# yifanlu0227/CoAlign

Hardware: AMD Instinct MI355X
Metric: frames_per_s_5agent_opv2v_synthetic (higher is better)
Workload: dtype f32 (3x3 convolutions: every operand rounded to 22 significant bits and split into two fp16 terms, the low term scaled by 2^10 and the weights by a per-output-channel power of two so that both terms are normal fp16 numbers at any scale; three fp16 matrix products per fp32 product, f32 accumulation

## Files before the change

coalign_amd/backbone.py:

```python
from __future__ import annotations

import os
from collections import namedtuple
from typing import List, Optional, Sequence

import torch
import torch.nn as nn
import torch.nn.functional as F

from . import ops

FAST_INFERENCE = True


def _bn(ch: int, eps: float) -> nn.BatchNorm2d:
    return nn.BatchNorm2d(ch, eps=eps, momentum=0.01)


def _fast_ok(module: nn.Module, x: torch.Tensor) -> bool:
    return FAST_INFERENCE and (not module.training) and x.is_cuda and x.dtype == torch.float32


HIP_CONV_POLICY = os.environ.get("COALIGN_HIP_CONV", "stage1")

# ... 7 lines not shown


def _terms(terms: Optional[int]) -> int:
    return CONV_EMU_TERMS if terms is None else terms


def emu_active(terms: Optional[int] = None) -> bool:
    return _terms(terms) in EMU_MODES

NHWC_STAGE_OUTPUTS = os.environ.get("COALIGN_NHWC_STAGES", "1") != "0"
CONV_EMU_TAP_MAJOR = os.environ.get("COALIGN_EMU_TAPK", "1") != "0"
CONV_WINOGRAD = os.environ.get("COALIGN_WINOGRAD", "0") != "0"


SPLIT_MAPS = os.environ.get("COALIGN_SPLIT_MAPS", "1") != "0"
HEAD_SPLIT_MAPS = os.environ.get("COALIGN_HEAD_SPLIT_MAPS", "1") != "0"


S2_SPLIT = os.environ.get("COALIGN_S2_SP", "all")
S2_SKIP = os.environ.get("COALIGN_S2_SKIP", "1") != "0"


HEADS_ONE_LAUNCH = os.environ.get("COALIGN_HEADS_ONE_LAUNCH", "1") != "0"
HEADS_SPLIT_IN = os.environ.get("COALIGN_HEADS_SP", "1") != "0"
COMPRESS_SPARSE = os.environ.get("COALIGN_COMPRESS_SPARSE", "1") != "0"


def split_maps_active(terms: Optional[int] = None) -> bool:
    return SPLIT_MAPS and _terms(terms) == 16 and NHWC_STAGE_OUTPUTS and CONV_EMU_TAP_MAJOR and POINTWISE_EMU


SP_MAX_COUT, SP_MAX_COUT_SKIP = 1024, 512


def sp_channels_ok(cin: Optional[int], cout: int, skip: bool = False) -> bool:
    return cout % 64 == 0 and 0 < cout <= (SP_MAX_COUT_SKIP if skip else SP_MAX_COUT) and (cin is None or (cin > 0 and cin % 16 == 0))


def narrow_channels_ok(cin: int, cout: int) -> bool:
    return cout in ops.NARROW_COUTS and cin > 0 and cin % 16 == 0


def winograd_active(terms: Optional[int] = None) -> bool:
    return CONV_WINOGRAD and _terms(terms) == 3 and NHWC_STAGE_OUTPUTS


# ... 368 lines not shown

    def _pointwise_ok(self, feats: Sequence[torch.Tensor]) -> bool:
        if not self.heads_pointwise() or not _fast_ok(self, feats[0]):
            return False
        sizes = {(f.shape[0], f.shape[2] * self.deblocks[i][0].stride[0], f.shape[3] * self.deblocks[i][0].stride[0]) for i, f in enumerate(feats[: self.num_levels])}
        return len(sizes) == 1

    def _upsample_concat(self, feats: Sequence[torch.Tensor], out_split: bool = False):
        if self._pointwise_ok(feats):
            ops_, c_tot = [], 0
            for i, f in enumerate(feats[: self.num_levels]):
                blk = self.deblocks[i]
                op, bn = blk[0], blk[1]
                w, b = _cache_of(blk, "_coalign_pw_cache").get(blk, lambda op=op, bn=bn: (lambda wf, bf: (PointwisePack(wf, True), bf))(*fold_bn(op.weight, None, bn, out_dim=1)))
                ops_.append((f, w, b, op.out_channels, op.stride[0], c_tot))
                c_tot += op.out_channels
            f0, s0 = feats[0], self.deblocks[0][0].stride[0]
            images = [w.get() for _, w, _, _, _, _ in ops_]
            if out_split and self.heads_write_split():
                x = ops.SplitMap.empty(f0.shape[0], c_tot, f0.shape[2] * s0, f0.shape[3] * s0, f0.device)
            else:
                x = torch.empty((f0.shape[0], c_tot, f0.shape[2] * s0, f0.shape[3] * s0), dtype=torch.float32, device=f0.device)
            if isinstance(x, ops.SplitMap) and HEADS_ONE_LAUNCH and 1 < len(ops_) <= 4:
                ops.pointwise_heads_split([(f, im, b, cout, up, off) for (f, w, b, cout, up, off), im in zip(ops_, images)], x)
            else:
                for (f, w, b, cout, up, off), im in zip(ops_, images):
                    ops.pointwise_conv(f, im, b, cout, up=up, relu=True, out=x, c_off=off)
        else:
            ups = [self._deblock(i, f) if len(self.deblocks) > 0 else f for i, f in enumerate(feats[: self.num_levels])]
            x = torch.cat(ups, dim=1) if len(ups) > 1 else ups[0]
        if len(self.deblocks) > self.num_levels:
            x = self._deblock(len(self.deblocks) - 1, x)
        return x

    def decode_multiscale_feature(self, feats: Sequence[torch.Tensor], out_split: bool = False):
        return self._upsample_concat(feats, out_split)

    def forward(self, data_dict: dict) -> dict:
        feats = self.get_multiscale_feature(data_dict["spatial_features"])
        data_dict["spatial_features_2d"] = self._upsample_concat(feats)
        return data_dict


def _backbone_cfg(model_cfg: dict):
    layer_nums, layer_strides, num_filters, ups, upf = (list(model_cfg.get(k, [])) for k in ("layer_nums", "layer_strides", "num_filters", "upsample_strides", "num_upsample_filter"))
    assert len(layer_nums) == len(layer_strides) == len(num_filters) and len(ups) == len(upf)
    return layer_nums, layer_strides, num_filters, ups, upf


class ResNetBEVBackbone(_MultiscaleDecodeMixin, nn.Module):
# ... 192 lines not shown
```

coalign_amd/csrc/pointwise.hip:

```cpp
#include "common.h"
#include <cstdlib>

namespace {

typedef float floatx16 __attribute__((ext_vector_type(16)));

constexpr int kMaxCin = 256;

struct PwArgs {
    const float *__restrict__ x, *__restrict__ w, *__restrict__ bias;
    float *__restrict__ y;
    int N, Cin, Hin, Win, in_stride, Hp, Wp, M, up, Cout, Ctot, c_off, relu;
    int in_nhwc;
    int pb;
    int out_nhwc;
    const unsigned long long *stamps;
    const int *tag_ptr;
    unsigned sparse_rows;
    int out_sp;
    int *range_flag;
};

template <int UP>
__device__ __forceinline__ void pw_store(const PwArgs &a, int n, int m0, bool second, int px, int half, const floatx16 &acc0, const floatx16 &acc1) {
    const int pixels = a.Hp * a.Wp;
    if (px >= pixels) return;
    const int hp = px / a.Wp, wp = px - hp * a.Wp;
    const int Ho = a.Hp * UP, Wo = a.Wp * UP;
    const size_t out_plane = (size_t)Ho * Wo;
    float *yout = a.y + ((size_t)n * a.Ctot + a.c_off) * out_plane;
#pragma unroll
    for (int t = 0; t < 2; ++t) {
        if (t == 1 && !second) break;
#pragma unroll
        for (int r4 = 0; r4 < 4; ++r4) {
            const int m = m0 + t * 32 + 8 * r4 + 4 * half;
            float v[4];
#pragma unroll
            for (int j = 0; j < 4; ++j) v[j] = t == 0 ? acc0[4 * r4 + j] : acc1[4 * r4 + j];
            if (UP == 4) {
                const int co = m >> 4, ky = (m >> 2) & 3;
                const float bb = a.bias[co];
                float4 o;
                o.x = v[0] + bb; o.y = v[1] + bb; o.z = v[2] + bb; o.w = v[3] + bb;
// ... 76 lines not shown
        }
    }
    __syncthreads();
    const int pbk = wave / WPB, rt = wave - pbk * WPB;
    const int m0 = m_base + rt * 64;
    const bool active = m0 < a.M;
    if (!active && !a.out_sp) return;
    const bool second = m0 + 32 < a.M;
    floatx16 acc0 = {0}, acc1 = {0};
    const float *w0 = a.w + m0 + p;
    const float *xb = xt + pbk * 32 + p;
#pragma unroll 8
    for (int k0 = 0; k0 < a.Cin; k0 += 2) {
        const float b = xb[(k0 + half) * TP];
        const float a0 = w0[(size_t)(k0 + half) * a.M];
        const float a1 = second ? w0[(size_t)(k0 + half) * a.M + 32] : 0.f;
        acc0 = __builtin_amdgcn_mfma_f32_32x32x2f32(a0, b, acc0, 0, 0, 0);
        acc1 = __builtin_amdgcn_mfma_f32_32x32x2f32(a1, b, acc1, 0, 0, 0);
    }
    pw_store<UP>(a, n, m0, second, p0 + pbk * 32 + p, half, acc0, acc1);
}

template <int UP>
__device__ __forceinline__ void pw_store_sp(const PwArgs &a, float *stage, int n, int m_base, int p0, int RW, int PB, int tid, int pbk, int rt, int lane, bool active, bool second,
                                            const floatx16 &acc0, const floatx16 &acc1) {
    constexpr int UU = UP * UP;
    const int half = lane >> 5, p = lane & 31;
    __syncthreads();
    if (active) {
#pragma unroll
        for (int t = 0; t < 2; ++t) {
            if (t == 1 && !second) break;
#pragma unroll
            for (int r = 0; r < 16; ++r) {
                const int row = rt * 64 + t * 32 + 8 * (r / 4) + 4 * half + r % 4;
                stage[(pbk * RW + row) * 33 + p] = t == 0 ? acc0[r] : acc1[r];
            }
        }
    }
    __syncthreads();
    const int pixels = a.Hp * a.Wp, Ho = a.Hp * UP, Wo = a.Wp * UP;
    const size_t HWo = (size_t)Ho * Wo;
    const int c8n = RW / (8 * UU);
    const int items = PB * c8n * UU * 32;
    uint4 *ysp = reinterpret_cast<uint4 *>(a.y);
    bool big = false;
    for (int it = tid; it < items; it += 256) {
        const int kx = it % UP, pp = (it / UP) & 31;
        int rest = it / (32 * UP);
        const int ky = rest % UP;
        rest /= UP;
        const int c8 = rest % c8n, pb = rest / c8n;
        const int co0 = m_base / UU + 8 * c8;
        const int px = p0 + pb * 32 + pp;
        if (co0 >= a.Cout || px >= pixels) continue;
        const int hp = px / a.Wp, wp = px - hp * a.Wp;
        const float4 b0 = *reinterpret_cast<const float4 *>(a.bias + co0), b1 = *reinterpret_cast<const float4 *>(a.bias + co0 + 4);
        const float bb[8] = {b0.x, b0.y, b0.z, b0.w, b1.x, b1.y, b1.z, b1.w};
        float v[8];
#pragma unroll
        for (int j = 0; j < 8; ++j) {
            v[j] = stage[(pb * RW + (8 * c8 + j) * UU + ky * UP + kx) * 33 + pp] + bb[j];
            if (a.relu) v[j] = fmaxf(v[j], 0.f);
            big = big || fabsf(v[j]) > 65504.f;
        }
        unsigned h[4], l[4];
#pragma unroll
        for (int k = 0; k < 4; ++k) coalign::sp16_split2(v[2 * k], v[2 * k + 1], h[k], l[k]);
        const int cg = a.c_off + co0;
        const size_t idx = ((size_t)(n * (a.Ctot / 16) + cg / 16) * 4 + ((cg >> 3) & 1) * 2) * HWo + (size_t)(hp * UP + ky) * Wo + wp * UP + kx;
        ysp[idx] = uint4{h[0], h[1], h[2], h[3]};
        ysp[idx + HWo] = uint4{l[0], l[1], l[2], l[3]};
    }
    if (a.range_flag && big) atomicOr(a.range_flag, 1);
}

typedef __bf16 bf16x8 __attribute__((ext_vector_type(8)));

__device__ __forceinline__ void split8(const float (&v)[8], bf16x8 (&out)[3]) {
#pragma unroll
    for (int i = 0; i < 8; ++i) {
        const __bf16 h = (__bf16)v[i];
        const float r = v[i] - (float)h;
        const __bf16 m = (__bf16)r;
        out[0][i] = h; out[1][i] = m; out[2][i] = (__bf16)(r - (float)m);
    }
}

template <int UP>
__device__ __forceinline__ void pointwise_emu_body(const PwArgs &a, uint4 *xs, int bx, int by, int bz) {
    const int tid = threadIdx.x, wave = tid >> 6, lane = tid & 63, half = lane >> 5, p = lane & 31;
    const int pixels = a.Hp * a.Wp;
    const int PB = a.pb, WPB = 4 / PB, TP = 32 * PB;
    const int p0 = bx * TP, n = bz;
    const int m_base = by * (64 * WPB);
    const size_t in_plane = (size_t)a.Hin * a.Win;
    const float *xin = a.stamps ? a.x : a.x + (size_t)n * a.Cin * in_plane;
    const int G = a.Cin >> 3;
    {
        const int pl = tid & (TP - 1), g0 = tid / TP, gstep = 256 / TP;
        const int px = p0 + pl;
        const bool ok0 = px < pixels;
        const int hp = ok0 ? px / a.Wp : 0, wp = ok0 ? px - hp * a.Wp : 0;
        size_t off = (size_t)(hp * a.in_stride) * a.Win + (size_t)wp * a.in_stride;
        bool ok = ok0;
        if (a.stamps) {
            const unsigned long long st = a.stamps[(size_t)n * in_plane + off];
            ok = ok0 && (unsigned)(st >> 32) == (unsigned)*a.tag_ptr && (unsigned)st < a.sparse_rows;
            off = ok ? (size_t)(unsigned)st : 0;
        }
        for (int g = g0; g < G; g += gstep) {
            float u[8];
            if (a.in_nhwc) {
                const float4 *xp = reinterpret_cast<const float4 *>(xin + off * a.Cin) + 2 * g;
                const float4 q0 = xp[0], q1 = xp[1];
                u[0] = q0.x; u[1] = q0.y; u[2] = q0.z; u[3] = q0.w; u[4] = q1.x; u[5] = q1.y; u[6] = q1.z; u[7] = q1.w;
            } else {
#pragma unroll
                for (int j = 0; j < 8; ++j) u[j] = xin[(size_t)(8 * g + j) * in_plane + off];
            }
            if (!ok) {
#pragma unroll
                for (int j = 0; j < 8; ++j) u[j] = 0.f;
            }
            bf16x8 o[3];
            split8(u, o);
#pragma unroll
            for (int t = 0; t < 3; ++t) xs[(t * G + g) * TP + pl] = __builtin_bit_cast(uint4, o[t]);
        }
    }
    __syncthreads();
    const int pbk = wave / WPB, rt = wave - pbk * WPB;
    const int m0 = m_base + rt * 64;
    const bool active = m0 < a.M;
    if (!active && !a.out_sp) return;
    const bool second = m0 + 32 < a.M;
    const int S = a.Cin >> 4;
    const uint4 *w0 = reinterpret_cast<const uint4 *>(a.w) + (size_t)((active ? m0 : 0) >> 5) * S * 192 + lane;
    const uint4 *w1 = w0 + (second ? (size_t)S * 192 : 0);
    const uint4 *xb = xs + pbk * 32 + p;
    floatx16 acc0 = {0}, acc1 = {0};
    constexpr int wi[6] = {0, 1, 2, 0, 1, 0};
    constexpr int bi[6] = {2, 1, 0, 1, 0, 0};
    bf16x8 wa[3], wb[3], bc[3];
#pragma unroll
    for (int t = 0; t < 3; ++t) {
        wa[t] = __builtin_bit_cast(bf16x8, w0[t * 64]);
        wb[t] = __builtin_bit_cast(bf16x8, w1[t * 64]);
        bc[t] = __builtin_bit_cast(bf16x8, xb[(t * G + half) * TP]);
    }
    const int steps = active ? S : 0;
#pragma unroll 2
    for (int s = 0; s < steps; ++s) {
        bf16x8 na[3], nb[3], nc[3];
        const int sn = s + 1 < S ? s + 1 : s;
#pragma unroll
        for (int t = 0; t < 3; ++t) {
            na[t] = __builtin_bit_cast(bf16x8, w0[(sn * 3 + t) * 64]);
            nb[t] = __builtin_bit_cast(bf16x8, w1[(sn * 3 + t) * 64]);
            nc[t] = __builtin_bit_cast(bf16x8, xb[(t * G + 2 * sn + half) * TP]);
        }
#pragma unroll
        for (int i = 0; i < 6; ++i) {
            acc0 = __builtin_amdgcn_mfma_f32_32x32x16_bf16(wa[wi[i]], bc[bi[i]], acc0, 0, 0, 0);
            acc1 = __builtin_amdgcn_mfma_f32_32x32x16_bf16(wb[wi[i]], bc[bi[i]], acc1, 0, 0, 0);
        }
#pragma unroll
        for (int t = 0; t < 3; ++t) { wa[t] = na[t]; wb[t] = nb[t]; bc[t] = nc[t]; }
    }
    if (a.out_sp) pw_store_sp<UP>(a, reinterpret_cast<float *>(xs), n, m_base, p0, 64 * WPB, PB, tid, pbk, rt, lane, active, second, acc0, acc1);
    else pw_store<UP>(a, n, m0, second, p0 + pbk * 32 + p, half, acc0, acc1);
}

template <int UP>
__global__ __launch_bounds__(256) void pointwise_emu_kernel(const PwArgs a) {
    extern __shared__ uint4 xs[];
    pointwise_emu_body<UP>(a, xs, blockIdx.x, blockIdx.y, blockIdx.z);
}

constexpr int kMultiMax = 4;
struct PwMulti {
    PwArgs l[kMultiMax];
    int first[kMultiMax + 1], gx[kMultiMax], gy[kMultiMax];
    int n;
};

__global__ __launch_bounds__(256) void pointwise_emu_multi_kernel(const PwMulti m) {
    extern __shared__ uint4 xs[];
    const int bid = blockIdx.x;
#define COALIGN_PW_SLOT(K)                                                                  \
    if (bid >= m.first[K] && bid < m.first[K + 1]) {                                        \
        const PwArgs &a = m.l[K];                                                           \
        const int local = bid - m.first[K], gx = m.gx[K], gy = m.gy[K];                     \
        const int bx = local % gx, by = (local / gx) % gy, bz = local / (gx * gy);          \
        if (a.up == 4) pointwise_emu_body<4>(a, xs, bx, by, bz);                            \
        else if (a.up == 2) pointwise_emu_body<2>(a, xs, bx, by, bz);                       \
        else pointwise_emu_body<1>(a, xs, bx, by, bz);                                      \
        return;                                                                             \
    }
    COALIGN_PW_SLOT(0)
    COALIGN_PW_SLOT(1)
    COALIGN_PW_SLOT(2)
    COALIGN_PW_SLOT(3)
#undef COALIGN_PW_SLOT
}

}

extern "C" int coalign_pointwise_conv(const float *x, const float *w, const float *bias, float *y, int N, int Cin, int Hin, int Win,
                                      int in_stride, int Cout, int up, int M_padded, int Ctot, int c_off, int relu, void *stream) {
    return coalign_pointwise_conv_ex(x, w, bias, y, N, Cin, Hin, Win, in_stride, Cout, up, M_padded, Ctot, c_off, relu, 0, stream);
}

static int pointwise_prepare(const float *x, const float *w, const float *bias, float *y, int N, int Cin, int Hin, int Win,
                             int in_stride, int Cout, int up, int M_padded, int Ctot, int c_off, int relu, int in_nhwc, bool emu,
                             const void *stamps, const int32_t *state, bool out_sp, int32_t *range_flag, int sparse_rows, PwArgs &a, dim3 &grid, size_t &lds) {
    using namespace coalign;
    if (!x || !w || !bias || !y) return COALIGN_ERR_NULL_POINTER;
    if (emu && ((Cin & 15) || (reinterpret_cast<uintptr_t>(w) & 15))) return COALIGN_ERR_UNSUPPORTED;
    if (N < 0 || Cin < 1 || Hin < 1 || Win < 1 || Cout < 1 || Ctot < Cout || c_off < 0 || c_off + Cout > Ctot) return COALIGN_ERR_BAD_SHAPE;
    if ((in_nhwc & 1) && ((Cin & 3) || (reinterpret_cast<uintptr_t>(x) & 15))) return COALIGN_ERR_UNSUPPORTED;
    if (Cin > (emu ? 2 * kMaxCin : kMaxCin) || (Cin & 1) || (up != 1 && up != 2 && up != 4) || (in_stride != 1 && in_stride != 2) || (up != 1 && in_stride != 1))
        return COALIGN_ERR_UNSUPPORTED;
    const int M = Cout * up * up;
    if (M_padded < M || M_padded % 32 || (up != 1 && M_padded != M)) return COALIGN_ERR_BAD_SHAPE;
    const int out_nhwc = (in_nhwc >> 1) & 1;
    in_nhwc &= 1;
    if (out_nhwc && (up != 1 || (Ctot & 3) || (c_off & 3) || ((reinterpret_cast<uintptr_t>(y) | reinterpret_cast<uintptr_t>(bias)) & 15))) return COALIGN_ERR_UNSUPPORTED;
    a = PwArgs{x, w, bias, y, N, Cin, Hin, Win, in_stride, (Hin + in_stride - 1) / in_stride, (Win + in_stride - 1) / in_stride, M_padded, up, Cout, Ctot, c_off, relu, in_nhwc != 0, 1, out_nhwc,
               static_cast<const unsigned long long *>(stamps), state, (unsigned)(sparse_rows < 0 ? 0 : sparse_rows), out_sp ? 1 : 0, range_flag};
    if (out_sp && (!emu || out_nhwc || (Cout & 15) || (Ctot & 15) || (c_off & 15) || (reinterpret_cast<uintptr_t>(y) & 15) || (reinterpret_cast<uintptr_t>(bias) & 15) ||
                   M_padded != Cout * up * up || (size_t)N * Ctot * a.Hp * up * a.Wp * up >= ((size_t)1 << 33)))
        return COALIGN_ERR_UNSUPPORTED;
    if (stamps && (!in_nhwc || !state || (reinterpret_cast<uintptr_t>(stamps) & 7))) return COALIGN_ERR_UNSUPPORTED;
    if (N > 65535) return COALIGN_ERR_UNSUPPORTED;
    const int pixels = a.Hp * a.Wp;
    static const int pb_max = coalign::lab_env("COALIGN_PW_PB", 4);
    a.pb = M_padded <= 64 ? 4 : M_padded <= 128 ? 2 : 1;
    while (a.pb > 1 && (a.pb > pb_max || Cin * 32 * a.pb > kMaxCin * 32)) a.pb >>= 1;
    if (up == 4 && ((a.Wp * 4) % 4 || (reinterpret_cast<uintptr_t>(y) & 15))) return COALIGN_ERR_UNSUPPORTED;
    if (up == 2 && (reinterpret_cast<uintptr_t>(y) & 7)) return COALIGN_ERR_UNSUPPORTED;
    const int rows_per_wg = 64 * (4 / a.pb), px_per_wg = 32 * a.pb;
    grid = dim3((pixels + px_per_wg - 1) / px_per_wg, (M_padded + rows_per_wg - 1) / rows_per_wg, N);
    lds = 0;
    if (emu) {
        lds = (size_t)Cin * px_per_wg * 6;
        if (out_sp && lds < (size_t)256 * 33 * 4) lds = (size_t)256 * 33 * 4;
    }
    return COALIGN_OK;
}

static int pointwise_big_lds(size_t lds) {
    using namespace coalign;
    static bool big_lds_dev[16] = {false};
    int dev = 0;
    if (hipGetDevice(&dev) != hipSuccess || dev < 0 || dev >= 16) dev = 0;
    bool &big_lds = big_lds_dev[dev];
    if (lds > 48 * 1024 && !big_lds) {
        const void *fns[4] = {reinterpret_cast<const void *>(pointwise_emu_kernel<1>), reinterpret_cast<const void *>(pointwise_emu_kernel<2>),
                              reinterpret_cast<const void *>(pointwise_emu_kernel<4>), reinterpret_cast<const void *>(pointwise_emu_multi_kernel)};
        for (const void *fn : fns) {
            const int rc = hip_call(hipFuncSetAttribute(fn, hipFuncAttributeMaxDynamicSharedMemorySize, 96 * 1024));
            if (rc != COALIGN_OK) {
                (void)hipGetLastError();
                return rc;
            }
        }
        big_lds = true;
    }
    return COALIGN_OK;
}

static int pointwise_impl(const float *x, const float *w, const float *bias, float *y, int N, int Cin, int Hin, int Win,
                          int in_stride, int Cout, int up, int M_padded, int Ctot, int c_off, int relu, int in_nhwc, bool emu,
                          void *stream, const void *stamps = nullptr, const int32_t *state = nullptr, bool out_sp = false, int32_t *range_flag = nullptr, int sparse_rows = 0) {
    using namespace coalign;
    PwArgs a;
    dim3 grid;
    size_t lds;
    int rc = pointwise_prepare(x, w, bias, y, N, Cin, Hin, Win, in_stride, Cout, up, M_padded, Ctot, c_off, relu, in_nhwc, emu, stamps, state, out_sp, range_flag, sparse_rows, a, grid, lds);
    if (rc != COALIGN_OK) return rc;
    if (N == 0) return COALIGN_OK;
    hipStream_t s = static_cast<hipStream_t>(stream);
    if (emu) {
        rc = pointwise_big_lds(lds);
        if (rc != COALIGN_OK) return rc;
        if (up == 4) hipLaunchKernelGGL(pointwise_emu_kernel<4>, grid, dim3(256), lds, s, a);
        else if (up == 2) hipLaunchKernelGGL(pointwise_emu_kernel<2>, grid, dim3(256), lds, s, a);
        else hipLaunchKernelGGL(pointwise_emu_kernel<1>, grid, dim3(256), lds, s, a);
        return check_launch();
    }
    if (up == 4) hipLaunchKernelGGL(pointwise_kernel<4>, grid, dim3(256), 0, s, a);
    else if (up == 2) hipLaunchKernelGGL(pointwise_kernel<2>, grid, dim3(256), 0, s, a);
    else hipLaunchKernelGGL(pointwise_kernel<1>, grid, dim3(256), 0, s, a);
    return check_launch();
}

extern "C" int coalign_pointwise_conv_ex(const float *x, const float *w, const float *bias, float *y, int N, int Cin, int Hin, int Win,
                                         int in_stride, int Cout, int up, int M_padded, int Ctot, int c_off, int relu, int in_nhwc,
                                         void *stream) {
    return pointwise_impl(x, w, bias, y, N, Cin, Hin, Win, in_stride, Cout, up, M_padded, Ctot, c_off, relu, in_nhwc, false, stream);
}

extern "C" size_t coalign_pointwise_emu_weight_bytes(int Cin, int M_padded) {
    if (Cin < 16 || (Cin & 15) || Cin > 2 * kMaxCin || M_padded < 32 || (M_padded & 31)) return 0;
    return (size_t)M_padded * Cin * 6;
}

extern "C" int coalign_pointwise_conv_emu(const float *x, const void *w_split, const float *bias, float *y, int N, int Cin, int Hin, int Win,
                                          int in_stride, int Cout, int up, int M_padded, int Ctot, int c_off, int relu, int in_nhwc,
                                          void *stream) {
    return pointwise_impl(x, static_cast<const float *>(w_split), bias, y, N, Cin, Hin, Win, in_stride, Cout, up, M_padded, Ctot, c_off, relu, in_nhwc,
                          true, stream);
}

extern "C" int coalign_pointwise_conv_emu_sparse(const float *feats, int M_rows, const void *stamps, const int32_t *state, const void *w_split, const float *bias, float *y,
                                                 int N, int Cin, int Hin, int Win, int Cout, int M_padded, int relu, int out_nhwc, void *stream) {
    if (!stamps || !state) return COALIGN_ERR_NULL_POINTER;
    if (M_rows < 0) return COALIGN_ERR_BAD_SHAPE;
    return pointwise_impl(feats, static_cast<const float *>(w_split), bias, y, N, Cin, Hin, Win, 2, Cout, 1, M_padded, Cout, 0, relu, 1 | (out_nhwc ? 2 : 0), true, stream,
                          stamps, state, false, nullptr, M_rows);
}

extern "C" int coalign_pointwise_conv_emu_sp(const float *x, const void *w_split, const float *bias, void *y_sp, int N, int Cin, int Hin, int Win, int in_stride,
                                             int Cout, int up, int M_padded, int Ctot, int c_off, int relu, int in_nhwc, int32_t *range_flag, void *stream) {
    if (in_nhwc & ~1) return COALIGN_ERR_UNSUPPORTED;
    return pointwise_impl(x, static_cast<const float *>(w_split), bias, static_cast<float *>(y_sp), N, Cin, Hin, Win, in_stride, Cout, up, M_padded, Ctot, c_off, relu, in_nhwc,
                          true, stream, nullptr, nullptr, true, range_flag);
}

extern "C" int coalign_pointwise_conv_emu_sp_multi(int n_layers, const void *const *x, const void *const *w_split, const void *const *bias, const int32_t *Cin, const int32_t *Hin,
                                                   const int32_t *Win, const int32_t *Cout, const int32_t *up, const int32_t *c_off, const int32_t *in_nhwc, void *y_sp, int N, int Ctot,
                                                   int relu, int32_t *range_flag, void *stream) {
    using namespace coalign;
    if (!x || !w_split || !bias || !Cin || !Hin || !Win || !Cout || !up || !c_off || !in_nhwc || !y_sp) return COALIGN_ERR_NULL_POINTER;
    if (n_layers < 1 || n_layers > kMultiMax) return COALIGN_ERR_UNSUPPORTED;
    PwMulti m{};
    m.n = n_layers;
    size_t lds = 0;
    int order[kMultiMax];
    long long work[kMultiMax];
    for (int i = 0; i < n_layers; ++i) {
        if (in_nhwc[i] & ~1) return COALIGN_ERR_UNSUPPORTED;
        if (Hin[i] * up[i] != Hin[0] * up[0] || Win[i] * up[i] != Win[0] * up[0]) return COALIGN_ERR_BAD_SHAPE;
        order[i] = i;
        work[i] = (long long)Cin[i] * Cout[i] * up[i] * up[i];
    }
    for (int i = 0; i < n_layers; ++i)
        for (int j = i + 1; j < n_layers; ++j)
            if (work[order[j]] > work[order[i]]) { const int t = order[i]; order[i] = order[j]; order[j] = t; }
    for (int k = 0; k < n_layers; ++k) {
        const int i = order[k];
        dim3 grid;
        size_t l;
        const int rc = pointwise_prepare(static_cast<const float *>(x[i]), static_cast<const float *>(w_split[i]), static_cast<const float *>(bias[i]), static_cast<float *>(y_sp), N, Cin[i],
                                         Hin[i], Win[i], 1, Cout[i], up[i], Cout[i] * up[i] * up[i], Ctot, c_off[i], relu, in_nhwc[i], true, nullptr, nullptr, true, range_flag, 0, m.l[k], grid, l);
        if (rc != COALIGN_OK) return rc;
        m.gx[k] = (int)grid.x;
        m.gy[k] = (int)grid.y;
        m.first[k + 1] = m.first[k] + (int)(grid.x * grid.y * grid.z);
        if (l > lds) lds = l;
    }
    for (int k = n_layers; k < kMultiMax; ++k) m.first[k + 1] = m.first[n_layers];
    if (N == 0) return COALIGN_OK;
    const int rc = pointwise_big_lds(lds);
    if (rc != COALIGN_OK) return rc;
    hipLaunchKernelGGL(pointwise_emu_multi_kernel, dim3(m.first[n_layers]), dim3(256), lds, static_cast<hipStream_t>(stream), m);
    return check_launch();
}

namespace {

typedef _Float16 hd_halfx8 __attribute__((ext_vector_type(8)));

struct HeadsArgs {
    const uint4 *__restrict__ x, *__restrict__ w;
    const float *__restrict__ winv, *__restrict__ bias;
    float *__restrict__ y;
    int N, Cin, HW, M;
};

constexpr int kHeadsAhead = 4;

__global__ __launch_bounds__(256) void heads_sp_kernel(const HeadsArgs a) {
    const int tid = threadIdx.x, wave = tid >> 6, lane = tid & 63, half = lane >> 5, p = lane & 31;
    const int n = blockIdx.y, px0 = (blockIdx.x * 4 + wave) * 32;
    if (px0 >= a.HW) return;
    const int px = px0 + p, pix = px < a.HW ? px : a.HW - 1;
    const int CI16 = a.Cin / 16;
    const uint4 *xb = a.x + ((size_t)n * CI16 * 4 + 2 * half) * a.HW + pix;
// ... 50 lines not shown
```

coalign_amd/ops.py:

```python
from __future__ import annotations

import ctypes
import os as _os
from typing import Optional, Sequence, Tuple

import numpy as np
import torch

from . import hip

FUSE_ATT, FUSE_MAX, FUSE_NONE = 0, 1, 2

PROFILE = None


def timed(name: str):
    return _Timed(name)


class _Timed:
    def __init__(self, name: str):
        self.name = name

    def __enter__(self):
# ... 1225 lines not shown
    co, ci = w.shape[0], w.shape[1]
    out = torch.zeros((ci, (co + 31) // 32 * 32), dtype=torch.float32, device=w.device)
    out[:, :co] = w.reshape(co, ci).t()
    return out


def pack_pointwise_emu_weight(w_packed: torch.Tensor) -> torch.Tensor:
    w = w_packed.detach().float()
    Cin, M = w.shape
    if Cin % 16 or M % 32:
        raise ValueError("pointwise emu weights: Cin % 16 == 0 and M % 32 == 0")
    h = w.to(torch.bfloat16)
    r1 = w - h.float()
    m = r1.to(torch.bfloat16)
    lo = (r1 - m.float()).to(torch.bfloat16)
    terms = torch.stack([h, m, lo], 0).view(torch.int16)
    img = terms.view(3, Cin // 16, 2, 8, M // 32, 32)
    img = img.permute(4, 1, 0, 2, 5, 3).contiguous()
    return img.view(M // 32, Cin // 16, 3, 64, 8)


@_device_op
def pointwise_conv(x: torch.Tensor, w_packed: torch.Tensor, bias: torch.Tensor, cout: int, up: int = 1, in_stride: int = 1, relu: bool = True,
                   out: Optional[torch.Tensor] = None, c_off: int = 0, out_channels_last: bool = False) -> torch.Tensor:
    _need_gpu(x, w_packed, bias)
    emu = w_packed.dtype == torch.int16
    L = hip.lib()
    nhwc = x.dtype == torch.float32 and is_channels_last(x) and x.shape[1] % 4 == 0
    xc = x if nhwc else _f32c(x)
    N, Cin, Hin, Win = xc.shape
    Ho, Wo = (Hin + in_stride - 1) // in_stride * up, (Win + in_stride - 1) // in_stride * up
    if isinstance(out, SplitMap):
        if not emu or out_channels_last or tuple(out.shape[2:]) != (Ho, Wo) or out.shape[0] != N or cout % 16 or c_off % 16 or c_off + cout > out.shape[1]:
            raise ValueError("SplitMap output: split-bf16 weight image, [N, Ctot, Ho, Wo] map, Cout and c_off multiples of 16")
        if w_packed.dim() != 5 or w_packed.shape[1] * 16 != Cin or not w_packed.is_contiguous() or w_packed.shape[0] * 32 != cout * up * up:
            raise ValueError("split weight image does not match (Cin, Cout * up * up)")
        with _Timed("pointwise_conv"):
            hip.check(L.coalign_pointwise_conv_emu_sp(_ptr(xc), _ptr(w_packed), _ptr(_f32c(bias)), _ptr(out.data), N, Cin, Hin, Win, in_stride, cout, up, w_packed.shape[0] * 32,
                                                      out.shape[1], c_off, int(relu), int(nhwc), _ptr(sp_range_flag(xc.device)), _stream()), "coalign_pointwise_conv_emu_sp")
        return out
    if out_channels_last:
        if out is not None or up != 1 or cout % 4:
            raise ValueError("channels-last output: up = 1, Cout % 4 == 0, no output slice")
        out = torch.empty((N, cout, Ho, Wo), dtype=torch.float32, device=xc.device, memory_format=torch.channels_last)
    elif out is None:
        out = torch.empty((N, cout, Ho, Wo), dtype=torch.float32, device=xc.device)
    if tuple(out.shape[2:]) != (Ho, Wo) or out.shape[0] != N or not (nhwc_memory(out) if out_channels_last else out.is_contiguous()) or out.dtype != torch.float32:
        raise ValueError("output buffer shape / layout mismatch")
    nhwc_flags = int(nhwc) | (2 if out_channels_last else 0)
    with _Timed("pointwise_conv"):
        if emu:
            if w_packed.dim() != 5 or w_packed.shape[1] * 16 != Cin or not w_packed.is_contiguous():
                raise ValueError("split weight image does not match Cin")
            hip.check(L.coalign_pointwise_conv_emu(_ptr(xc), _ptr(w_packed), _ptr(_f32c(bias)), _ptr(out), N, Cin, Hin, Win, in_stride, cout, up,
                                                   w_packed.shape[0] * 32, out.shape[1], c_off, int(relu), nhwc_flags, _stream()), "coalign_pointwise_conv_emu")
        else:
            hip.check(L.coalign_pointwise_conv_ex(_ptr(xc), _ptr(w_packed), _ptr(_f32c(bias)), _ptr(out), N, Cin, Hin, Win, in_stride, cout, up,
                                                  w_packed.shape[1], out.shape[1], c_off, int(relu), nhwc_flags, _stream()), "coalign_pointwise_conv")
    return out


@_device_op
def pointwise_heads_split(layers, out: "SplitMap", relu: bool = True) -> "SplitMap":
    L = hip.lib()
    n = len(layers)
    N = out.shape[0]
    keep, xs, ws, bs = [], [], [], []
    ci, hi, wi, co, ups, offs, nh = [], [], [], [], [], [], []
    for (x, w_emu, bias, cout, up, c_off) in layers:
        _need_gpu(x, w_emu, bias)
        nhwc = x.dtype == torch.float32 and is_channels_last(x) and x.shape[1] % 4 == 0
        xc = x if nhwc else _f32c(x)
        b = _f32c(bias)
        if w_emu.dtype != torch.int16 or w_emu.dim() != 5 or w_emu.shape[1] * 16 != xc.shape[1] or not w_emu.is_contiguous() or w_emu.shape[0] * 32 != cout * up * up or xc.shape[0] != N:
            raise ValueError("pointwise_heads_split: split weight image of (Cin, Cout * up * up), one batch size")
        keep += [xc, b]
        xs.append(xc.data_ptr()); ws.append(w_emu.data_ptr()); bs.append(b.data_ptr())
        ci.append(xc.shape[1]); hi.append(xc.shape[2]); wi.append(xc.shape[3]); co.append(cout); ups.append(up); offs.append(c_off); nh.append(int(nhwc))
    arr_p = lambda v: (ctypes.c_void_p * n)(*v)
    arr_i = lambda v: (ctypes.c_int32 * n)(*v)
    with _Timed("pointwise_heads_split"):
        hip.check(L.coalign_pointwise_conv_emu_sp_multi(n, arr_p(xs), arr_p(ws), arr_p(bs), arr_i(ci), arr_i(hi), arr_i(wi), arr_i(co), arr_i(ups), arr_i(offs), arr_i(nh), _ptr(out.data),
                                                        N, out.shape[1], int(relu), _ptr(sp_range_flag(out.device)), _stream()), "coalign_pointwise_conv_emu_sp_multi")
    return out


HEADS_SP_MAX_ROWS = 32


def pack_heads_sp_weight(weight: torch.Tensor) -> torch.Tensor:
    w = weight.detach().float().reshape(weight.shape[0], weight.shape[1])
    if w.shape[0] > HEADS_SP_MAX_ROWS:
        raise ValueError("heads_sp serves at most 32 head channels")
    pad = torch.zeros((64, w.shape[1]), dtype=torch.float32, device=w.device)
    pad[: w.shape[0]] = w
    return pack_conv1x1_sp_weight(pad)


@_device_op
def heads_sp(x: "SplitMap", w_sp: torch.Tensor, bias: torch.Tensor, M: int) -> torch.Tensor:
    if not isinstance(x, SplitMap):
# ... 157 lines not shown
```

Before: 691.0.

## Add 2x2 register-tiled pointwise emu kernel with chunked input staging for upsample heads

Adds a new pointwise (1x1/deconv) emulated-fp32 kernel that computes a 2x2 MFMA tile per wave (two row blocks by two pixel blocks), reusing each loaded weight fragment across two pixel groups. It stages input channels into LDS in chunks of KC slices rather than all at once, and is enabled by default for the upsample/concat heads through a flag bit. This raises the arithmetic done per weight load and lowers LDS footprint, at the cost of more accumulator registers and extra barriers between chunks. Optional trace instrumentation macros are also added behind a compile flag.

```diff
diff --git a/coalign_amd/backbone.py b/coalign_amd/backbone.py
--- a/coalign_amd/backbone.py
+++ b/coalign_amd/backbone.py
@@ -53,6 +53,7 @@
 
 
 HEADS_ONE_LAUNCH = os.environ.get("COALIGN_HEADS_ONE_LAUNCH", "1") != "0"
+UPHEADS_TILE = os.environ.get("COALIGN_UPHEADS_TILE", "1") != "0"
 HEADS_SPLIT_IN = os.environ.get("COALIGN_HEADS_SP", "1") != "0"
 COMPRESS_SPARSE = os.environ.get("COALIGN_COMPRESS_SPARSE", "1") != "0"
 
@@ -467,10 +468,10 @@
             else:
                 x = torch.empty((f0.shape[0], c_tot, f0.shape[2] * s0, f0.shape[3] * s0), dtype=torch.float32, device=f0.device)
             if isinstance(x, ops.SplitMap) and HEADS_ONE_LAUNCH and 1 < len(ops_) <= 4:
-                ops.pointwise_heads_split([(f, im, b, cout, up, off) for (f, w, b, cout, up, off), im in zip(ops_, images)], x)
+                ops.pointwise_heads_split([(f, im, b, cout, up, off) for (f, w, b, cout, up, off), im in zip(ops_, images)], x, tile=UPHEADS_TILE)
             else:
                 for (f, w, b, cout, up, off), im in zip(ops_, images):
-                    ops.pointwise_conv(f, im, b, cout, up=up, relu=True, out=x, c_off=off)
+                    ops.pointwise_conv(f, im, b, cout, up=up, relu=True, out=x, c_off=off, tile=UPHEADS_TILE)
         else:
             ups = [self._deblock(i, f) if len(self.deblocks) > 0 else f for i, f in enumerate(feats[: self.num_levels])]
             x = torch.cat(ups, dim=1) if len(ups) > 1 else ups[0]
diff --git a/coalign_amd/csrc/pointwise.hip b/coalign_amd/csrc/pointwise.hip
--- a/coalign_amd/csrc/pointwise.hip
+++ b/coalign_amd/csrc/pointwise.hip
@@ -19,7 +19,48 @@
     unsigned sparse_rows;
     int out_sp;
     int *range_flag;
+    int kc;
+#ifdef PW_TRACE
+    long long *trace;
+    int trace_lds;
+#endif
 };
+
+#ifdef PW_TRACE
+#define PW_TRACE_INIT()                                                                                                          \
+    long long *pw_tr = reinterpret_cast<long long *>(reinterpret_cast<char *>(xs) + a.trace_lds) + wave * 64;                  \
+    const bool pw_on = a.trace && bx == ((pixels + TP - 1) / TP) / 2 && by == 0 && bz == 0;                                      \
+    if (pw_on) pw_tr[lane] = 0
+#define PW_STAMP(k)                                                                                                              \
+    do {                                                                                                                         \
+        unsigned long long pw_t;                                                                                                 \
+        __builtin_amdgcn_sched_barrier(0);                                                                                       \
+        asm volatile("s_memtime %0\n\ts_waitcnt lgkmcnt(0)" : "=s"(pw_t)::"memory");                                            \
+        __builtin_amdgcn_sched_barrier(0);                                                                                       \
+        if (pw_on && lane == 0 && (k) < 64) pw_tr[k] = (long long)pw_t;                                                          \
+    } while (0)
+#define PW_STEP_WAIT(s)                                                                                                          \
+    do {                                                                                                                         \
+        if ((s) < 19) PW_STAMP(2 + 2 * (s));                                                                                     \
+        asm volatile("s_waitcnt vmcnt(6)" ::: "memory");        \
+        if ((s) < 19) PW_STAMP(3 + 2 * (s));                                                                                     \
+    } while (0)
+#define PW_TRACE_FLUSH()                                                                                                         \
+    do {                                                                                                                         \
+        asm volatile("s_waitcnt vmcnt(0)" ::: "memory");                                                                         \
+        PW_STAMP(44);                                                                                                            \
+        if (pw_on) a.trace[((a.up >> 1) * 4 + wave) * 64 + lane] = pw_tr[lane];                                                  \
+    } while (0)
+#define PW_TRACE_PARAMS , bool pw_on, long long *pw_tr
+#define PW_TRACE_ARGS , pw_on, pw_tr
+#else
+#define PW_TRACE_INIT() (void)0
+#define PW_STAMP(k) (void)0
+#define PW_STEP_WAIT(s) (void)0
+#define PW_TRACE_FLUSH() (void)0
+#define PW_TRACE_PARAMS
+#define PW_TRACE_ARGS
+#endif
 
 template <int UP>
 __device__ __forceinline__ void pw_store(const PwArgs &a, int n, int m0, bool second, int px, int half, const floatx16 &acc0, const floatx16 &acc1) {
@@ -142,23 +183,8 @@
 }
 
 template <int UP>
-__device__ __forceinline__ void pw_store_sp(const PwArgs &a, float *stage, int n, int m_base, int p0, int RW, int PB, int tid, int pbk, int rt, int lane, bool active, bool second,
-                                            const floatx16 &acc0, const floatx16 &acc1) {
+__device__ __forceinline__ void pw_sp_groups(const PwArgs &a, const float *stage, int n, int m_base, int p0, int RW, int PB, int tid) {
     constexpr int UU = UP * UP;
-    const int half = lane >> 5, p = lane & 31;
-    __syncthreads();
-    if (active) {
-#pragma unroll
-        for (int t = 0; t < 2; ++t) {
-            if (t == 1 && !second) break;
-#pragma unroll
-            for (int r = 0; r < 16; ++r) {
-                const int row = rt * 64 + t * 32 + 8 * (r / 4) + 4 * half + r % 4;
-                stage[(pbk * RW + row) * 33 + p] = t == 0 ? acc0[r] : acc1[r];
-            }
-        }
-    }
-    __syncthreads();
     const int pixels = a.Hp * a.Wp, Ho = a.Hp * UP, Wo = a.Wp * UP;
     const size_t HWo = (size_t)Ho * Wo;
     const int c8n = RW / (8 * UU);
@@ -195,6 +221,29 @@
     if (a.range_flag && big) atomicOr(a.range_flag, 1);
 }
 
+template <int UP>
+__device__ __forceinline__ void pw_store_sp(const PwArgs &a, float *stage, int n, int m_base, int p0, int RW, int PB, int tid, int pbk, int rt, int lane, bool active, bool second,
+                                            const floatx16 &acc0, const floatx16 &acc1 PW_TRACE_PARAMS) {
+    const int half = lane >> 5, p = lane & 31;
+    __syncthreads();
+    PW_STAMP(41);
+    if (active) {
+#pragma unroll
+        for (int t = 0; t < 2; ++t) {
+            if (t == 1 && !second) break;
+#pragma unroll
+            for (int r = 0; r < 16; ++r) {
+                const int row = rt * 64 + t * 32 + 8 * (r / 4) + 4 * half + r % 4;
+                stage[(pbk * RW + row) * 33 + p] = t == 0 ? acc0[r] : acc1[r];
+            }
+        }
+    }
+    PW_STAMP(42);
+    __syncthreads();
+    PW_STAMP(43);
+    pw_sp_groups<UP>(a, stage, n, m_base, p0, RW, PB, tid);
+}
+
 typedef __bf16 bf16x8 __attribute__((ext_vector_type(8)));
 
 __device__ __forceinline__ void split8(const float (&v)[8], bf16x8 (&out)[3]) {
@@ -217,6 +266,8 @@
     const size_t in_plane = (size_t)a.Hin * a.Win;
     const float *xin = a.stamps ? a.x : a.x + (size_t)n * a.Cin * in_plane;
     const int G = a.Cin >> 3;
+    PW_TRACE_INIT();
+    PW_STAMP(0);
     {
         const int pl = tid & (TP - 1), g0 = tid / TP, gstep = 256 / TP;
         const int px = p0 + pl;
@@ -250,6 +301,7 @@
         }
     }
     __syncthreads();
+    PW_STAMP(1);
     const int pbk = wave / WPB, rt = wave - pbk * WPB;
     const int m0 = m_base + rt * 64;
     const bool active = m0 < a.M;
@@ -278,8 +330,10 @@
         for (int t = 0; t < 3; ++t) {
             na[t] = __builtin_bit_cast(bf16x8, w0[(sn * 3 + t) * 64]);
             nb[t] = __builtin_bit_cast(bf16x8, w1[(sn * 3 + t) * 64]);
-            nc[t] = __builtin_bit_cast(bf16x8, xb[(t * G + 2 * sn + half) * TP]);
-        }
+        }
+        PW_STEP_WAIT(s);
+#pragma unroll
+        for (int t = 0; t < 3; ++t) nc[t] = __builtin_bit_cast(bf16x8, xb[(t * G + 2 * sn + half) * TP]);
 #pragma unroll
         for (int i = 0; i < 6; ++i) {
             acc0 = __builtin_amdgcn_mfma_f32_32x32x16_bf16(wa[wi[i]], bc[bi[i]], acc0, 0, 0, 0);
@@ -288,8 +342,129 @@
 #pragma unroll
         for (int t = 0; t < 3; ++t) { wa[t] = na[t]; wb[t] = nb[t]; bc[t] = nc[t]; }
     }
-    if (a.out_sp) pw_store_sp<UP>(a, reinterpret_cast<float *>(xs), n, m_base, p0, 64 * WPB, PB, tid, pbk, rt, lane, active, second, acc0, acc1);
-    else pw_store<UP>(a, n, m0, second, p0 + pbk * 32 + p, half, acc0, acc1);
+    PW_STAMP(40);
+    if (a.out_sp) {
+        pw_store_sp<UP>(a, reinterpret_cast<float *>(xs), n, m_base, p0, 64 * WPB, PB, tid, pbk, rt, lane, active, second, acc0, acc1 PW_TRACE_ARGS);
+        PW_TRACE_FLUSH();
+    } else {
+        pw_store<UP>(a, n, m0, second, p0 + pbk * 32 + p, half, acc0, acc1);
+    }
+}
+
+template <int UP>
+__device__ __forceinline__ void pointwise_emu_tile_body(const PwArgs &a, uint4 *xs, int bx, int by, int bz) {
+    const int tid = threadIdx.x, wave = tid >> 6, lane = tid & 63, half = lane >> 5, p = lane & 31;
+    const int pixels = a.Hp * a.Wp;
+    const int PP = a.pb, RT = 4 / PP, TP = 64 * PP;
+    const int p0 = bx * TP, n = bz, m_base = by * (64 * RT);
+    const int pq = wave / RT, rt = wave - pq * RT;
+    const int m0 = m_base + rt * 64;
+    const bool active = m0 < a.M, second = m0 + 32 < a.M;
+    const int S = a.Cin >> 4, KC = a.kc, GC = 2 * KC;
+    const size_t in_plane = (size_t)a.Hin * a.Win;
+    const float *xin = a.x + (size_t)n * a.Cin * in_plane;
+    PW_TRACE_INIT();
+    PW_STAMP(0);
+    const int pl = tid & (TP - 1), g0 = tid / TP, gstep = 256 / TP;
+    const bool ok = p0 + pl < pixels;
+    const int hp = ok ? (p0 + pl) / a.Wp : 0, wp = ok ? p0 + pl - hp * a.Wp : 0;
+    const size_t off = (size_t)(hp * a.in_stride) * a.Win + (size_t)wp * a.in_stride;
+    const uint4 *w0 = reinterpret_cast<const uint4 *>(a.w) + (size_t)((active ? m0 : 0) >> 5) * S * 192 + lane;
+    const uint4 *w1 = w0 + (second ? (size_t)S * 192 : 0);
+    const uint4 *xb = xs + pq * 64 + p;
+    floatx16 acc[2][2] = {{{0}, {0}}, {{0}, {0}}};
+    constexpr int wi[6] = {0, 1, 2, 0, 1, 0};
+    constexpr int bi[6] = {2, 1, 0, 1, 0, 0};
+    bf16x8 wa[3], wb[3], bc[2][3];
+#pragma unroll
+    for (int t = 0; t < 3; ++t) {
+        wa[t] = __builtin_bit_cast(bf16x8, w0[t * 64]);
+        wb[t] = __builtin_bit_cast(bf16x8, w1[t * 64]);
+    }
+    for (int s0 = 0; s0 < S; s0 += KC) {
+        const int ns = S - s0 < KC ? S - s0 : KC;
+        if (s0) {
+            if (s0 == KC) PW_STAMP(45);
+            __syncthreads();
+        }
+        for (int g = g0; g < 2 * ns; g += gstep) {
+            float u[8];
+            if (a.in_nhwc) {
+                const float4 *xp = reinterpret_cast<const float4 *>(xin + off * a.Cin) + 2 * (2 * s0 + g);
+                const float4 q0 = xp[0], q1 = xp[1];
+                u[0] = q0.x; u[1] = q0.y; u[2] = q0.z; u[3] = q0.w; u[4] = q1.x; u[5] = q1.y; u[6] = q1.z; u[7] = q1.w;
+            } else {
+#pragma unroll
+                for (int j = 0; j < 8; ++j) u[j] = xin[(size_t)(8 * (2 * s0 + g) + j) * in_plane + off];
+            }
+            if (!ok) {
+#pragma unroll
+                for (int j = 0; j < 8; ++j) u[j] = 0.f;
+            }
+            bf16x8 o[3];
+            split8(u, o);
+#pragma unroll
+            for (int t = 0; t < 3; ++t) xs[(t * GC + g) * TP + pl] = __builtin_bit_cast(uint4, o[t]);
+        }
+        __syncthreads();
+        if (s0 == 0) PW_STAMP(1);
+        if (s0 == KC) PW_STAMP(46);
+        if (!active) continue;
+#pragma unroll
+        for (int t = 0; t < 3; ++t) {
+            bc[0][t] = __builtin_bit_cast(bf16x8, xb[(t * GC + half) * TP]);
+            bc[1][t] = __builtin_bit_cast(bf16x8, xb[(t * GC + half) * TP + 32]);
+        }
+#pragma unroll 2
+        for (int s = 0; s < ns; ++s) {
+            bf16x8 na[3], nb[3], nc[2][3];
+            const int sn = s0 + s + 1 < S ? s0 + s + 1 : s0 + s;
+            const int ln = s + 1 < ns ? s + 1 : s;
+#pragma unroll
+            for (int t = 0; t < 3; ++t) {
+                na[t] = __builtin_bit_cast(bf16x8, w0[(sn * 3 + t) * 64]);
+                nb[t] = __builtin_bit_cast(bf16x8, w1[(sn * 3 + t) * 64]);
+            }
+            PW_STEP_WAIT(s0 + s);
+#pragma unroll
+            for (int t = 0; t < 3; ++t) {
+                nc[0][t] = __builtin_bit_cast(bf16x8, xb[(t * GC + 2 * ln + half) * TP]);
+                nc[1][t] = __builtin_bit_cast(bf16x8, xb[(t * GC + 2 * ln + half) * TP + 32]);
+            }
+#pragma unroll
+            for (int i = 0; i < 6; ++i) {
+                acc[0][0] = __builtin_amdgcn_mfma_f32_32x32x16_bf16(wa[wi[i]], bc[0][bi[i]], acc[0][0], 0, 0, 0);
+                acc[1][0] = __builtin_amdgcn_mfma_f32_32x32x16_bf16(wb[wi[i]], bc[0][bi[i]], acc[1][0], 0, 0, 0);
+                acc[0][1] = __builtin_amdgcn_mfma_f32_32x32x16_bf16(wa[wi[i]], bc[1][bi[i]], acc[0][1], 0, 0, 0);
+                acc[1][1] = __builtin_amdgcn_mfma_f32_32x32x16_bf16(wb[wi[i]], bc[1][bi[i]], acc[1][1], 0, 0, 0);
+            }
+#pragma unroll
+            for (int t = 0; t < 3; ++t) { wa[t] = na[t]; wb[t] = nb[t]; bc[0][t] = nc[0][t]; bc[1][t] = nc[1][t]; }
+        }
+    }
+    PW_STAMP(40);
+    float *stage = reinterpret_cast<float *>(xs);
+    const int RW = 64 * RT;
+    __syncthreads();
+    PW_STAMP(41);
+    if (active) {
+#pragma unroll
+        for (int t = 0; t < 2; ++t) {
+            if (t == 1 && !second) break;
+#pragma unroll
+            for (int q = 0; q < 2; ++q)
+#pragma unroll
+                for (int r = 0; r < 16; ++r) {
+                    const int row = rt * 64 + t * 32 + 8 * (r / 4) + 4 * half + r % 4;
+                    stage[((2 * pq + q) * RW + row) * 33 + p] = acc[t][q][r];
+                }
+        }
+    }
+    PW_STAMP(42);
+    __syncthreads();
+    PW_STAMP(43);
+    pw_sp_groups<UP>(a, stage, n, m_base, p0, RW, 2 * PP, tid);
+    PW_TRACE_FLUSH();
 }
 
 template <int UP>
@@ -308,20 +483,35 @@
 __global__ __launch_bounds__(256) void pointwise_emu_multi_kernel(const PwMulti m) {
     extern __shared__ uint4 xs[];
     const int bid = blockIdx.x;
-#define COALIGN_PW_SLOT(K)                                                                  \
+#define COALIGN_PW_SLOT(K, BODY)                                                            \
     if (bid >= m.first[K] && bid < m.first[K + 1]) {                                        \
         const PwArgs &a = m.l[K];                                                           \
         const int local = bid - m.first[K], gx = m.gx[K], gy = m.gy[K];                     \
         const int bx = local % gx, by = (local / gx) % gy, bz = local / (gx * gy);          \
-        if (a.up == 4) pointwise_emu_body<4>(a, xs, bx, by, bz);                            \
-        else if (a.up == 2) pointwise_emu_body<2>(a, xs, bx, by, bz);                       \
-        else pointwise_emu_body<1>(a, xs, bx, by, bz);                                      \
+        if (a.up == 4) BODY<4>(a, xs, bx, by, bz);                                          \
+        else if (a.up == 2) BODY<2>(a, xs, bx, by, bz);                                     \
+        else BODY<1>(a, xs, bx, by, bz);                                                    \
         return;                                                                             \
     }
-    COALIGN_PW_SLOT(0)
-    COALIGN_PW_SLOT(1)
-    COALIGN_PW_SLOT(2)
-    COALIGN_PW_SLOT(3)
+    COALIGN_PW_SLOT(0, pointwise_emu_body)
+    COALIGN_PW_SLOT(1, pointwise_emu_body)
+    COALIGN_PW_SLOT(2, pointwise_emu_body)
+    COALIGN_PW_SLOT(3, pointwise_emu_body)
+}
+
+template <int UP>
+__global__ __launch_bounds__(256) void pointwise_emu_tile_kernel(const PwArgs a) {
+    extern __shared__ uint4 xs[];
+    pointwise_emu_tile_body<UP>(a, xs, blockIdx.x, blockIdx.y, blockIdx.z);
+}
+
+__global__ __launch_bounds__(256) void pointwise_emu_tile_multi_kernel(const PwMulti m) {
+    extern __shared__ uint4 xs[];
+    const int bid = blockIdx.x;
+    COALIGN_PW_SLOT(0, pointwise_emu_tile_body)
+    COALIGN_PW_SLOT(1, pointwise_emu_tile_body)
+    COALIGN_PW_SLOT(2, pointwise_emu_tile_body)
+    COALIGN_PW_SLOT(3, pointwise_emu_tile_body)
 #undef COALIGN_PW_SLOT
 }
 
@@ -332,9 +522,14 @@
     return coalign_pointwise_conv_ex(x, w, bias, y, N, Cin, Hin, Win, in_stride, Cout, up, M_padded, Ctot, c_off, relu, 0, stream);
 }
 
+#ifdef PW_TRACE
+static long long *g_pw_trace = nullptr;
+extern "C" void coalign_pointwise_set_trace(long long *p) { g_pw_trace = p; }
+#endif
+
 static int pointwise_prepare(const float *x, const float *w, const float *bias, float *y, int N, int Cin, int Hin, int Win,
                              int in_stride, int Cout, int up, int M_padded, int Ctot, int c_off, int relu, int in_nhwc, bool emu,
-                             const void *stamps, const int32_t *state, bool out_sp, int32_t *range_flag, int sparse_rows, PwArgs &a, dim3 &grid, size_t &lds) {
+                             const void *stamps, const int32_t *state, bool out_sp, int32_t *range_flag, int sparse_rows, PwArgs &a, dim3 &grid, size_t &lds, bool tile = false) {
     using namespace coalign;
     if (!x || !w || !bias || !y) return COALIGN_ERR_NULL_POINTER;
     if (emu && ((Cin & 15) || (reinterpret_cast<uintptr_t>(w) & 15))) return COALIGN_ERR_UNSUPPORTED;
@@ -360,13 +555,28 @@
     while (a.pb > 1 && (a.pb > pb_max || Cin * 32 * a.pb > kMaxCin * 32)) a.pb >>= 1;
     if (up == 4 && ((a.Wp * 4) % 4 || (reinterpret_cast<uintptr_t>(y) & 15))) return COALIGN_ERR_UNSUPPORTED;
     if (up == 2 && (reinterpret_cast<uintptr_t>(y) & 7)) return COALIGN_ERR_UNSUPPORTED;
-    const int rows_per_wg = 64 * (4 / a.pb), px_per_wg = 32 * a.pb;
-    grid = dim3((pixels + px_per_wg - 1) / px_per_wg, (M_padded + rows_per_wg - 1) / rows_per_wg, N);
-    lds = 0;
-    if (emu) {
-        lds = (size_t)Cin * px_per_wg * 6;
-        if (out_sp && lds < (size_t)256 * 33 * 4) lds = (size_t)256 * 33 * 4;
-    }
+    if (tile) {
+        if (!out_sp || stamps) return COALIGN_ERR_UNSUPPORTED;
+        a.pb = M_padded <= 64 ? 4 : M_padded <= 128 ? 2 : 1;
+        const int rows = 64 * (4 / a.pb), px = 64 * a.pb;
+        a.kc = 512 / px;
+        if (a.kc > Cin / 16) a.kc = Cin / 16;
+        grid = dim3((pixels + px - 1) / px, (M_padded + rows - 1) / rows, N);
+        lds = (size_t)512 * 33 * 4;
+    } else {
+        const int rows_per_wg = 64 * (4 / a.pb), px_per_wg = 32 * a.pb;
+        grid = dim3((pixels + px_per_wg - 1) / px_per_wg, (M_padded + rows_per_wg - 1) / rows_per_wg, N);
+        lds = 0;
+        if (emu) {
+            lds = (size_t)Cin * px_per_wg * 6;
+            if (out_sp && lds < (size_t)256 * 33 * 4) lds = (size_t)256 * 33 * 4;
+        }
+    }
+#ifdef PW_TRACE
+    a.trace = g_pw_trace;
+    a.trace_lds = (int)lds;
+    if (emu) lds += 4 * 64 * sizeof(long long);
+#endif
     return COALIGN_OK;
 }
 
@@ -377,8 +587,10 @@
     if (hipGetDevice(&dev) != hipSuccess || dev < 0 || dev >= 16) dev = 0;
     bool &big_lds = big_lds_dev[dev];
     if (lds > 48 * 1024 && !big_lds) {
-        const void *fns[4] = {reinterpret_cast<const void *>(pointwise_emu_kernel<1>), reinterpret_cast<const void *>(pointwise_emu_kernel<2>),
-                              reinterpret_cast<const void *>(pointwise_emu_kernel<4>), reinterpret_cast<const void *>(pointwise_emu_multi_kernel)};
+        const void *fns[8] = {reinterpret_cast<const void *>(pointwise_emu_kernel<1>), reinterpret_cast<const void *>(pointwise_emu_kernel<2>),
+                              reinterpret_cast<const void *>(pointwise_emu_kernel<4>), reinterpret_cast<const void *>(pointwise_emu_multi_kernel),
+                              reinterpret_cast<const void *>(pointwise_emu_tile_kernel<1>), reinterpret_cast<const void *>(pointwise_emu_tile_kernel<2>),
+                              reinterpret_cast<const void *>(pointwise_emu_tile_kernel<4>), reinterpret_cast<const void *>(pointwise_emu_tile_multi_kernel)};
         for (const void *fn : fns) {
             const int rc = hip_call(hipFuncSetAttribute(fn, hipFuncAttributeMaxDynamicSharedMemorySize, 96 * 1024));
             if (rc != COALIGN_OK) {
@@ -393,18 +605,25 @@
 
 static int pointwise_impl(const float *x, const float *w, const float *bias, float *y, int N, int Cin, int Hin, int Win,
                           int in_stride, int Cout, int up, int M_padded, int Ctot, int c_off, int relu, int in_nhwc, bool emu,
-                          void *stream, const void *stamps = nullptr, const int32_t *state = nullptr, bool out_sp = false, int32_t *range_flag = nullptr, int sparse_rows = 0) {
+                          void *stream, const void *stamps = nullptr, const int32_t *state = nullptr, bool out_sp = false, int32_t *range_flag = nullptr, int sparse_rows = 0,
+                          bool tile = false) {
     using namespace coalign;
     PwArgs a;
     dim3 grid;
     size_t lds;
-    int rc = pointwise_prepare(x, w, bias, y, N, Cin, Hin, Win, in_stride, Cout, up, M_padded, Ctot, c_off, relu, in_nhwc, emu, stamps, state, out_sp, range_flag, sparse_rows, a, grid, lds);
+    int rc = pointwise_prepare(x, w, bias, y, N, Cin, Hin, Win, in_stride, Cout, up, M_padded, Ctot, c_off, relu, in_nhwc, emu, stamps, state, out_sp, range_flag, sparse_rows, a, grid, lds, tile);
     if (rc != COALIGN_OK) return rc;
     if (N == 0) return COALIGN_OK;
     hipStream_t s = static_cast<hipStream_t>(stream);
     if (emu) {
         rc = pointwise_big_lds(lds);
         if (rc != COALIGN_OK) return rc;
+        if (tile) {
+            if (up == 4) hipLaunchKernelGGL(pointwise_emu_tile_kernel<4>, grid, dim3(256), lds, s, a);
+            else if (up == 2) hipLaunchKernelGGL(pointwise_emu_tile_kernel<2>, grid, dim3(256), lds, s, a);
+            else hipLaunchKernelGGL(pointwise_emu_tile_kernel<1>, grid, dim3(256), lds, s, a);
+            return check_launch();
+        }
         if (up == 4) hipLaunchKernelGGL(pointwise_emu_kernel<4>, grid, dim3(256), lds, s, a);
         else if (up == 2) hipLaunchKernelGGL(pointwise_emu_kernel<2>, grid, dim3(256), lds, s, a);
         else hipLaunchKernelGGL(pointwise_emu_kernel<1>, grid, dim3(256), lds, s, a);
@@ -444,9 +663,9 @@
 
 extern "C" int coalign_pointwise_conv_emu_sp(const float *x, const void *w_split, const float *bias, void *y_sp, int N, int Cin, int Hin, int Win, int in_stride,
                                              int Cout, int up, int M_padded, int Ctot, int c_off, int relu, int in_nhwc, int32_t *range_flag, void *stream) {
-    if (in_nhwc & ~1) return COALIGN_ERR_UNSUPPORTED;
-    return pointwise_impl(x, static_cast<const float *>(w_split), bias, static_cast<float *>(y_sp), N, Cin, Hin, Win, in_stride, Cout, up, M_padded, Ctot, c_off, relu, in_nhwc,
-                          true, stream, nullptr, nullptr, true, range_flag);
+    if (in_nhwc & ~5) return COALIGN_ERR_UNSUPPORTED;
+    return pointwise_impl(x, static_cast<const float *>(w_split), bias, static_cast<float *>(y_sp), N, Cin, Hin, Win, in_stride, Cout, up, M_padded, Ctot, c_off, relu, in_nhwc & 1,
+                          true, stream, nullptr, nullptr, true, range_flag, 0, (in_nhwc & 4) != 0);
 }
 
 extern "C" int coalign_pointwise_conv_emu_sp_multi(int n_layers, const void *const *x, const void *const *w_split, const void *const *bias, const int32_t *Cin, const int32_t *Hin,
@@ -457,11 +676,12 @@
     if (n_layers < 1 || n_layers > kMultiMax) return COALIGN_ERR_UNSUPPORTED;
     PwMulti m{};
     m.n = n_layers;
+    const bool tile = (in_nhwc[0] & 4) != 0;
     size_t lds = 0;
     int order[kMultiMax];
     long long work[kMultiMax];
     for (int i = 0; i < n_layers; ++i) {
-        if (in_nhwc[i] & ~1) return COALIGN_ERR_UNSUPPORTED;
+        if ((in_nhwc[i] & ~5) || ((in_nhwc[i] ^ in_nhwc[0]) & 4)) return COALIGN_ERR_UNSUPPORTED;
         if (Hin[i] * up[i] != Hin[0] * up[0] || Win[i] * up[i] != Win[0] * up[0]) return COALIGN_ERR_BAD_SHAPE;
         order[i] = i;
         work[i] = (long long)Cin[i] * Cout[i] * up[i] * up[i];
@@ -474,7 +694,7 @@
         dim3 grid;
         size_t l;
         const int rc = pointwise_prepare(static_cast<const float *>(x[i]), static_cast<const float *>(w_split[i]), static_cast<const float *>(bias[i]), static_cast<float *>(y_sp), N, Cin[i],
-                                         Hin[i], Win[i], 1, Cout[i], up[i], Cout[i] * up[i] * up[i], Ctot, c_off[i], relu, in_nhwc[i], true, nullptr, nullptr, true, range_flag, 0, m.l[k], grid, l);
+                                         Hin[i], Win[i], 1, Cout[i], up[i], Cout[i] * up[i] * up[i], Ctot, c_off[i], relu, in_nhwc[i] & 1, true, nullptr, nullptr, true, range_flag, 0, m.l[k], grid, l, tile);
         if (rc != COALIGN_OK) return rc;
         m.gx[k] = (int)grid.x;
         m.gy[k] = (int)grid.y;
@@ -485,7 +705,8 @@
     if (N == 0) return COALIGN_OK;
     const int rc = pointwise_big_lds(lds);
     if (rc != COALIGN_OK) return rc;
-    hipLaunchKernelGGL(pointwise_emu_multi_kernel, dim3(m.first[n_layers]), dim3(256), lds, static_cast<hipStream_t>(stream), m);
+    if (tile) hipLaunchKernelGGL(pointwise_emu_tile_multi_kernel, dim3(m.first[n_layers]), dim3(256), lds, static_cast<hipStream_t>(stream), m);
+    else hipLaunchKernelGGL(pointwise_emu_multi_kernel, dim3(m.first[n_layers]), dim3(256), lds, static_cast<hipStream_t>(stream), m);
     return check_launch();
 }
 
diff --git a/coalign_amd/ops.py b/coalign_amd/ops.py
--- a/coalign_amd/ops.py
+++ b/coalign_amd/ops.py
@@ -1271,7 +1271,7 @@
 
 @_device_op
 def pointwise_conv(x: torch.Tensor, w_packed: torch.Tensor, bias: torch.Tensor, cout: int, up: int = 1, in_stride: int = 1, relu: bool = True,
-                   out: Optional[torch.Tensor] = None, c_off: int = 0, out_channels_last: bool = False) -> torch.Tensor:
+                   out: Optional[torch.Tensor] = None, c_off: int = 0, out_channels_last: bool = False, tile: bool = True) -> torch.Tensor:
     _need_gpu(x, w_packed, bias)
     emu = w_packed.dtype == torch.int16
     L = hip.lib()
@@ -1286,7 +1286,7 @@
             raise ValueError("split weight image does not match (Cin, Cout * up * up)")
         with _Timed("pointwise_conv"):
             hip.check(L.coalign_pointwise_conv_emu_sp(_ptr(xc), _ptr(w_packed), _ptr(_f32c(bias)), _ptr(out.data), N, Cin, Hin, Win, in_stride, cout, up, w_packed.shape[0] * 32,
-                                                      out.shape[1], c_off, int(relu), int(nhwc), _ptr(sp_range_flag(xc.device)), _stream()), "coalign_pointwise_conv_emu_sp")
+                                                      out.shape[1], c_off, int(relu), int(nhwc) | (4 if tile else 0), _ptr(sp_range_flag(xc.device)), _stream()), "coalign_pointwise_conv_emu_sp")
         return out
     if out_channels_last:
         if out is not None or up != 1 or cout % 4:
@@ -1310,7 +1310,7 @@
 
 
 @_device_op
-def pointwise_heads_split(layers, out: "SplitMap", relu: bool = True) -> "SplitMap":
+def pointwise_heads_split(layers, out: "SplitMap", relu: bool = True, tile: bool = True) -> "SplitMap":
     L = hip.lib()
     n = len(layers)
     N = out.shape[0]
@@ -1325,7 +1325,7 @@
             raise ValueError("pointwise_heads_split: split weight image of (Cin, Cout * up * up), one batch size")
         keep += [xc, b]
         xs.append(xc.data_ptr()); ws.append(w_emu.data_ptr()); bs.append(b.data_ptr())
-        ci.append(xc.shape[1]); hi.append(xc.shape[2]); wi.append(xc.shape[3]); co.append(cout); ups.append(up); offs.append(c_off); nh.append(int(nhwc))
+        ci.append(xc.shape[1]); hi.append(xc.shape[2]); wi.append(xc.shape[3]); co.append(cout); ups.append(up); offs.append(c_off); nh.append(int(nhwc) | (4 if tile else 0))
     arr_p = lambda v: (ctypes.c_void_p * n)(*v)
     arr_i = lambda v: (ctypes.c_int32 * n)(*v)
     with _Timed("pointwise_heads_split"):
```

After: 696.2, median of 6. No clear change (+0.8%).
